# VinAIResearch/COMBAT

Hardware: AMD Instinct MI355X
Metric: images/sec per alternated generator+surrogate step, CIFAR-10 bs=128, 1/2/4/8 GPU (higher is better)
Workload: dtype bf16; 1 GPU; train_generator.py --dataset cifar10 --pc 0.5 --noise_rate 0.08: alternated PreActResNet18 surrogate + UNet generator step (Phase C + Phase G, both Nesterov-SGD updates), bs=128 per GPU, on-device augmentation on; per_gpu_batch=128, global_batch=128, parallelism=dp1 (RCCL all-reduce of netC grads in Phase C, netG grads in Phase G), losses_finite=True, deterministic=True

## Files before the change

### combat_amd/csrc/common.hpp

```cpp
#pragma once
#include <hip/hip_runtime.h>
#include <hip/hip_ext.h>
#include <stdint.h>

#include "combat_hip.h"

typedef __attribute__((ext_vector_type(8))) __bf16 bf16x8_t;
typedef __attribute__((ext_vector_type(4))) float f32x4_t;
typedef __attribute__((ext_vector_type(4))) short s16x4_t;
typedef __attribute__((ext_vector_type(4))) unsigned int u32x4_t;

namespace combat_launch {
extern thread_local hipEvent_t t_stop;
extern thread_local bool t_stop_used;
}
#define COMBAT_LAUNCH(kernel, grid, block, smem, stream, ...)                                             \
    do {                                                                                                  \
        if (hipEvent_t stop_ = combat_launch::t_stop) {                                                   \
            hipExtLaunchKernelGGL(kernel, grid, block, smem, stream, nullptr, stop_, 0, __VA_ARGS__);     \
            combat_launch::t_stop_used = true;                                                            \
        } else {                                                                                          \
            hipLaunchKernelGGL(kernel, grid, block, smem, stream, __VA_ARGS__);                           \
        }                                                                                                 \
    } while (0)
// ... 33 lines not shown
    v[4] = bf16_bits_to_f32(u[2] & 0xffffu);
    v[5] = bf16_bits_to_f32(u[2] >> 16);
    v[6] = bf16_bits_to_f32(u[3] & 0xffffu);
    v[7] = bf16_bits_to_f32(u[3] >> 16);
}

__device__ __forceinline__ u32x4_t pack8v(const float (&v)[8]) {
    u32x4_t u;
    u[0] = pack_bf16x2(v[0], v[1]);
    u[1] = pack_bf16x2(v[2], v[3]);
    u[2] = pack_bf16x2(v[4], v[5]);
    u[3] = pack_bf16x2(v[6], v[7]);
    return u;
}

__device__ __forceinline__ uint4 pack8(const float (&v)[8]) {
    uint4 u;
    u.x = pack_bf16x2(v[0], v[1]);
    u.y = pack_bf16x2(v[2], v[3]);
    u.z = pack_bf16x2(v[4], v[5]);
    u.w = pack_bf16x2(v[6], v[7]);
    return u;
}

__device__ __forceinline__ void load8f(const float *p, float (&v)[8]) {
    const float4 a = *reinterpret_cast<const float4 *>(p);
    const float4 b = *reinterpret_cast<const float4 *>(p + 4);
    v[0] = a.x; v[1] = a.y; v[2] = a.z; v[3] = a.w;
    v[4] = b.x; v[5] = b.y; v[6] = b.z; v[7] = b.w;
}

__device__ __forceinline__ float round_bf16(float f) { return bf16_bits_to_f32(f32_to_bf16_bits(f)); }

__device__ __forceinline__ uint4 hilo_pixel(float r, float g, float b) {
    const float hr = round_bf16(r), hg = round_bf16(g), hb = round_bf16(b);
    uint4 u;
    u.x = pack_bf16x2(hr, hg);
    u.y = pack_bf16x2(hb, r - hr);
    u.z = pack_bf16x2(g - hg, b - hb);
    u.w = 0;
    return u;
}

static inline hipStream_t as_stream(void *s) { return reinterpret_cast<hipStream_t>(s); }

bool combat_deterministic();
float *combat_stream_scratch(void *stream, size_t bytes);

static inline int ilog2_exact(int v) {
    if (v <= 0 || (v & (v - 1))) return -1;
    int s = 0;
    while ((1 << s) < v) ++s;
    return s;
}
```

### combat_amd/csrc/conv_wgrad.hip

```cpp
#include "conv_common.hpp"
#include "plan.hpp"

namespace {

struct WgradParams {
    combat_wgrad_args a;
    int M, PQ, ntaps, tiles_k, tiles_c, split, pix_per_split;
    float *ws;
};

template <int BMC, int BNC>
struct WCfg {
    static constexpr int WGK = (BNC == 16) ? 4 : (BMC == 16 ? 1 : 2);
    static constexpr int WGC = 4 / WGK;
    static constexpr int WK = BMC / WGK;
    static constexpr int WC = BNC / WGC;
    static constexpr int FK = WK / 16;
    static constexpr int FC = WC / 16;
    static constexpr int SK = (BMC + 16) * 2;
    static constexpr int SC = (BNC + 16) * 2;
    static constexpr int CHK = BMC / 8;
    static constexpr int CHC = BNC / 8;
    static constexpr int ITK = (64 * CHK + 255) / 256;
    static constexpr int ITC = (64 * CHC + 255) / 256;
// ... 168 lines not shown
#pragma unroll
        for (int i = 0; i < T::FK; ++i)
#pragma unroll
            for (int j = 0; j < T::FC; ++j) {
                const int col = wave_c * T::WC + j * 16 + fr;
                const int row = wave_k * T::WK + i * 16 + fq * 4;
#pragma unroll
                for (int e = 0; e < 4; ++e) ep[(row + e) * T::EPS + col] = acc[i][j][e];
            }
    }
    __syncthreads();
    if (p.ws) {
        float *slab = p.ws + ((((size_t)sp * p.ntaps + tap) * p.tiles_k + tile_k) * p.tiles_c + tile_c) * (size_t)(BMC * BNC);
        for (int idx = tid; idx < BMC * BNC; idx += 256) {
            const int row = idx / BNC, col = idx - row * BNC;
            slab[idx] = ep[row * T::EPS + col];
        }
        return;
    }
    const int creal = a.c_real;
    for (int idx = tid; idx < BMC * BNC; idx += 256) {
        const int row = idx / BNC, col = idx - row * BNC;
        const int n = k0 + row;
        int c = c0 + col;
        if (n >= a.k_real || c >= C) continue;
        if (creal < C) {
            if (c >= 2 * creal) continue;
            if (c >= creal) c -= creal;
        }
        atomicAdd(a.dw + ((size_t)n * p.ntaps + tap) * creal + c, ep[row * T::EPS + col]);
    }
}

__global__ __launch_bounds__(256) void conv_wgrad_c8_kernel(const WgradParams p) {
    constexpr int BMC = 64, NCOL = 80, SK = (BMC + 16) * 2, SC = (NCOL + 16) * 2, BUF = 64 * (SK + SC);
    constexpr int CHK = BMC / 8, CHC = NCOL / 8, ITK = (64 * CHK + 255) / 256, ITC = (64 * CHC + 255) / 256;
    constexpr int FC = NCOL / 16, EPS = NCOL + 4;
    extern __shared__ __attribute__((aligned(16))) unsigned char smem[];
    const combat_wgrad_args &a = p.a;
    const int tid = threadIdx.x, lane = tid & 63, wid = tid >> 6;
    int bid = blockIdx.x;
    const int tile_k = bid % p.tiles_k;
    const int sp = bid / p.tiles_k;
    const int k0 = tile_k * BMC;
    const int m_begin = sp * p.pix_per_split;
    int m_end = m_begin + p.pix_per_split;
    if (m_end > p.M) m_end = p.M;
    const int nkt = (m_end - m_begin + 63) / 64;
    if (nkt <= 0) return;
    const __bf16 *__restrict__ src = reinterpret_cast<const __bf16 *>(a.src);
    const __bf16 *__restrict__ dy = reinterpret_cast<const __bf16 *>(a.dy);
    const int K = a.K, H = a.H, W = a.W;
    u32x4_t rk[ITK];
    uint4 rc[ITC];
    auto load_tile = [&](int kt) {
        const int mt = m_begin + kt * 64;
#pragma unroll
        for (int i = 0; i < ITK; ++i) {
            const int idx = tid + 256 * i;
            const int row = idx / CHK, ch = idx % CHK;
            const int m = mt + row;
            u32x4_t v = {0u, 0u, 0u, 0u};
            if (idx < 64 * CHK && m < m_end) v = *reinterpret_cast<const u32x4_t *>(dy + (size_t)m * K + k0 + ch * 8);
            rk[i] = v;
        }
#pragma unroll
        for (int i = 0; i < ITC; ++i) {
            const int idx = tid + 256 * i;
            const int row = idx / CHC, tap = idx % CHC;
            const int m = mt + row;
            uint4 v = make_uint4(0, 0, 0, 0);
            if (idx < 64 * CHC && m < m_end && tap < 9) {
                const int img = m / p.PQ, rem = m - img * p.PQ;
                const int oy = rem / a.Q, ox = rem - oy * a.Q;
                const int r = (tap * 11) >> 5, s = tap - r * 3;
                const int iy = oy * a.stride - a.pad + r, ix = ox * a.stride - a.pad + s;
                if ((unsigned)iy < (unsigned)H && (unsigned)ix < (unsigned)W)
                    v = *reinterpret_cast<const uint4 *>(src + ((size_t)(img * H + iy) * W + ix) * 8);
            }
            rc[i] = v;
        }
    };
    auto store_tile = [&](int buf) {
        unsigned char *kl = smem + buf * BUF;
        unsigned char *cl = kl + 64 * SK;
#pragma unroll
        for (int i = 0; i < ITK; ++i) {
            const int idx = tid + 256 * i;
            if (idx < 64 * CHK) *reinterpret_cast<u32x4_t *>(kl + (idx / CHK) * SK + (idx % CHK) * 16) = rk[i];
        }
#pragma unroll
        for (int i = 0; i < ITC; ++i) {
            const int idx = tid + 256 * i;
            if (idx < 64 * CHC) *reinterpret_cast<uint4 *>(cl + (idx / CHC) * SC + (idx % CHC) * 16) = rc[i];
        }
    };
    f32x4_t acc[FC];
#pragma unroll
    for (int j = 0; j < FC; ++j) acc[j] = f32x4_t{0.f, 0.f, 0.f, 0.f};
    auto compute = [&](int buf) {
        const unsigned char *kl = smem + buf * BUF;
        const unsigned char *cl = kl + 64 * SK;
        const int q = (lane & 15) >> 2, pp = lane & 3, fq = lane >> 4;
        typedef __attribute__((ext_vector_type(8))) short s16x8_t;
        bf16x8_t fk[2], fc[2][FC];
#pragma unroll
        for (int ks = 0; ks < 2; ++ks) {
            const int prow = ks * 32 + fq * 8 + q;
            {
                const unsigned char *b = kl + prow * SK + (wid * 16 + pp * 4) * 2;
                const s16x4_t lo = lds_tr16(b), hi = lds_tr16(b + 4 * SK);
                const s16x8_t v = {lo[0], lo[1], lo[2], lo[3], hi[0], hi[1], hi[2], hi[3]};
                fk[ks] = __builtin_bit_cast(bf16x8_t, v);
            }
#pragma unroll
            for (int j = 0; j < FC; ++j) {
                const unsigned char *b = cl + prow * SC + (j * 16 + pp * 4) * 2;
                const s16x4_t lo = lds_tr16(b), hi = lds_tr16(b + 4 * SC);
                const s16x8_t v = {lo[0], lo[1], lo[2], lo[3], hi[0], hi[1], hi[2], hi[3]};
                fc[ks][j] = __builtin_bit_cast(bf16x8_t, v);
            }
        }
        __builtin_amdgcn_sched_barrier(0);
#pragma unroll
        for (int ks = 0; ks < 2; ++ks)
#pragma unroll
            for (int j = 0; j < FC; ++j) acc[j] = __builtin_amdgcn_mfma_f32_16x16x32_bf16(fk[ks], fc[ks][j], acc[j], 0, 0, 0);
        __builtin_amdgcn_sched_barrier(0);
    };
    load_tile(0);
    store_tile(0);
    __syncthreads();
    for (int kt = 0; kt < nkt; ++kt) {
        const bool more = kt + 1 < nkt;
        if (more) load_tile(kt + 1);
        compute(kt & 1);
        if (more) store_tile((kt + 1) & 1);
        __syncthreads();
    }
    float *ep = reinterpret_cast<float *>(smem);
    {
        const int fr = lane & 15, fq = lane >> 4;
#pragma unroll
        for (int j = 0; j < FC; ++j) {
            const int col = j * 16 + fr, row = wid * 16 + fq * 4;
#pragma unroll
            for (int e = 0; e < 4; ++e) ep[(row + e) * EPS + col] = acc[j][e];
        }
    }
    __syncthreads();
    const int creal = a.c_real;
    if (p.ws) {
        float *slab = p.ws + (size_t)blockIdx.x * (BMC * 9 * creal);
        for (int idx = tid; idx < BMC * 9 * creal; idx += 256) {
            const int row = idx / (9 * creal), rem = idx - row * 9 * creal;
            const int tap = rem / creal, c = rem - tap * creal;
            float v = ep[row * EPS + tap * 8 + c];
            if (creal < 8 && c + creal < 8) v += ep[row * EPS + tap * 8 + c + creal];
            slab[idx] = v;
        }
        return;
    }
    for (int idx = tid; idx < BMC * 72; idx += 256) {
        const int row = idx / 72, col = idx - row * 72;
        const int n = k0 + row, tap = col >> 3;
        int c = col & 7;
        if (n >= a.k_real) continue;
        if (creal < 8) {
            if (c >= 2 * creal) continue;
            if (c >= creal) c -= creal;
        }
        atomicAdd(a.dw + ((size_t)n * 9 + tap) * creal + c, ep[row * EPS + col]);
    }
}

__global__ __launch_bounds__(256) void conv_wgrad_c8_reduce_kernel(const float *__restrict__ ws, float *__restrict__ dw,
                                                                   int tiles_k, int split, int per_tile, int k_real,
                                                                   int row_elems, float *__restrict__ part) {
    const int e = blockIdx.x * 256 + threadIdx.x, tile_k = blockIdx.y;
    if (e >= per_tile) return;
    const int n = tile_k * 64 + e / row_elems;
    if (n >= k_real) return;
    float s0 = 0.f, s1 = 0.f, s2 = 0.f, s3 = 0.f;
    const int G = gridDim.z;
    int sp = blockIdx.z;
    for (; sp + 3 * G < split; sp += 4 * G) {
        s0 += ws[((size_t)sp * tiles_k + tile_k) * per_tile + e];
        s1 += ws[((size_t)(sp + G) * tiles_k + tile_k) * per_tile + e];
        s2 += ws[((size_t)(sp + 2 * G) * tiles_k + tile_k) * per_tile + e];
        s3 += ws[((size_t)(sp + 3 * G) * tiles_k + tile_k) * per_tile + e];
    }
    for (; sp < split; sp += G) s0 += ws[((size_t)sp * tiles_k + tile_k) * per_tile + e];
    const float s = (s0 + s1) + (s2 + s3);
    if (part) part[((size_t)blockIdx.z * tiles_k + tile_k) * per_tile + e] = s;
    else atomicAdd(dw + (size_t)tile_k * per_tile + e, s);
}

int launch_c8(WgradParams p, hipStream_t st) {
    constexpr int SMEM = 2 * 64 * ((64 + 16) * 2 + (80 + 16) * 2);
    static_assert(SMEM >= 64 * 84 * 4, "epilogue image");
    static bool attr_set = false;
    if (!attr_set) {
        if (hipFuncSetAttribute(reinterpret_cast<const void *>(conv_wgrad_c8_kernel), hipFuncAttributeMaxDynamicSharedMemorySize, SMEM) != hipSuccess)
            return COMBAT_ELAUNCH;
        attr_set = true;
    }
    p.tiles_k = p.a.K / 64;
    p.tiles_c = 1;
    int split = p.a.split;
    const int ktiles = (p.M + 63) / 64;
    if (split <= 0) {
        split = (256 + p.tiles_k - 1) / p.tiles_k;
        const int max_split = (ktiles + 3) / 4;
        if (split > max_split) split = max_split;
        if (split < 1) split = 1;
    }
    if (split > ktiles) split = ktiles;
    p.pix_per_split = ((ktiles + split - 1) / split) * 64;
    p.split = (p.M + p.pix_per_split - 1) / p.pix_per_split;
    const int per_tile = 64 * 9 * p.a.c_real;
    const long need = (long)p.tiles_k * p.split * per_tile * 4;
    p.ws = (p.split > 1 && p.a.workspace && p.a.workspace_bytes >= need) ? reinterpret_cast<float *>(p.a.workspace) : nullptr;
    if (combat_deterministic() && p.split > 1 && !p.ws) return COMBAT_EINVAL;
    COMBAT_LAUNCH(conv_wgrad_c8_kernel, dim3((unsigned)(p.tiles_k * p.split)), dim3(256), SMEM, st, p);
    CB_LAUNCH_CHECK();
    if (p.ws) {
        const int groups = p.split >= 32 ? 16 : 1;
        float *part = nullptr;
        if (combat_deterministic() && groups > 1) {
            const long extra = (long)groups * p.tiles_k * per_tile * 4;
            if (p.a.workspace_bytes >= need + extra) part = p.ws + need / 4;
        }
        const int g1 = combat_deterministic() && !part ? 1 : groups;
        COMBAT_LAUNCH(conv_wgrad_c8_reduce_kernel, dim3((per_tile + 255) / 256, p.tiles_k, g1), dim3(256), 0, st, (const float *)p.ws,
                           p.a.dw, p.tiles_k, p.split, per_tile, p.a.k_real, 9 * p.a.c_real, part);
        CB_LAUNCH_CHECK();
        if (part) {
            COMBAT_LAUNCH(conv_wgrad_c8_reduce_kernel, dim3((per_tile + 255) / 256, p.tiles_k, 1), dim3(256), 0, st, (const float *)part,
                               p.a.dw, p.tiles_k, groups, per_tile, p.a.k_real, 9 * p.a.c_real, (float *)nullptr);
            CB_LAUNCH_CHECK();
        }
    }
    return COMBAT_OK;
}

__global__ __launch_bounds__(256) void wgrad_slab_reduce_kernel(const float *__restrict__ ws, float *__restrict__ dw, int split,
                                                                int ntaps, int tiles_k, int tiles_c, int bmc, int bnc, int k_real,
                                                                int c_real, int C) {
    const long e = (long)blockIdx.x * 256 + threadIdx.x;
    if (e >= (long)k_real * ntaps * c_real) return;
    const int c = (int)(e % c_real), tap = (int)((e / c_real) % ntaps), n = (int)(e / ((long)c_real * ntaps));
    const int tile_k = n / bmc, row = n - tile_k * bmc;
    const size_t tile_elems = (size_t)bmc * bnc, sstride = (size_t)ntaps * tiles_k * tiles_c * tile_elems;
    float total = 0.f;
    for (int half = 0; half < 2; ++half) {
        const int cs = c + half * c_real;
        if (half && (c_real >= C || cs >= C || cs >= 2 * c_real)) break;
        const int tile_c = cs / bnc, col = cs - tile_c * bnc;
        const float *src = ws + (((size_t)tap * tiles_k + tile_k) * tiles_c + tile_c) * tile_elems + (size_t)row * bnc + col;
        float s0 = 0.f, s1 = 0.f, s2 = 0.f, s3 = 0.f;
        int sp = 0;
        for (; sp + 4 <= split; sp += 4) {
            s0 += src[(size_t)sp * sstride];
            s1 += src[(size_t)(sp + 1) * sstride];
            s2 += src[(size_t)(sp + 2) * sstride];
            s3 += src[(size_t)(sp + 3) * sstride];
        }
        for (; sp < split; ++sp) s0 += src[(size_t)sp * sstride];
        total += (s0 + s1) + (s2 + s3);
    }
    dw[e] += total;
}
// ... 39 lines not shown
    COMBAT_LAUNCH(kern, dim3((unsigned)blocks), dim3(256), T::SMEM, st, p);
    CB_LAUNCH_CHECK();
    if (p.ws) {
        const long elems = (long)p.a.k_real * p.ntaps * p.a.c_real;
        COMBAT_LAUNCH(wgrad_slab_reduce_kernel, dim3((unsigned)((elems + 255) / 256)), dim3(256), 0, st, (const float *)p.ws, p.a.dw,
                      p.split, p.ntaps, p.tiles_k, p.tiles_c, BMC, BNC, p.a.k_real, p.a.c_real, p.a.C);
        CB_LAUNCH_CHECK();
    }
    return COMBAT_OK;
}

template <int BMC, int BNC>
int generic_split(const combat_wgrad_args &a) {
    const long M = (long)a.N * a.P * a.Q;
    const int ktiles = (int)((M + 63) / 64), ntaps = a.R * a.S;
    const int tiles_k = (a.K + BMC - 1) / BMC, tiles_c = (a.C + BNC - 1) / BNC;
    int split = a.split > 0 ? a.split : 0;
    if (split <= 0) {
        const int base = tiles_k * tiles_c * ntaps;
        split = ((BMC == 16 ? 2304 : 256) + base - 1) / base;
        const int max_split = (ktiles + 3) / 4;
        if (split > max_split) split = max_split;
        if (split < 1) split = 1;
    }
    if (split > ktiles) split = ktiles;
    const int pix_per_split = ((ktiles + split - 1) / split) * 64;
    return (int)((M + pix_per_split - 1) / pix_per_split);
}

bool c8_applies(const combat_wgrad_args *a) {
    return a->split >= 0 && a->C == 8 && a->R == 3 && (a->K & 63) == 0 && !a->pro_scale && !a->pro_act;
}

int64_t c8_workspace(const combat_wgrad_args &a) {
    const long M = (long)a.N * a.P * a.Q;
    const int ktiles = (int)((M + 63) / 64), tiles_k = a.K / 64;
    int split = a.split;
    if (split <= 0) {
        split = (256 + tiles_k - 1) / tiles_k;
        const int max_split = (ktiles + 3) / 4;
        if (split > max_split) split = max_split;
        if (split < 1) split = 1;
    }
    if (split > ktiles) split = ktiles;
    const int pix_per_split = ((ktiles + split - 1) / split) * 64;
    const long nsplit = (M + pix_per_split - 1) / pix_per_split;
    if (nsplit <= 1) return 0;
    const int64_t per_tile = 64 * 9 * a.c_real * 4;
    return tiles_k * nsplit * per_tile + (nsplit >= 32 ? 16 * tiles_k * per_tile : 0);
}

int64_t generic_workspace(const combat_wgrad_args &a) {
    if (a.C <= 16) return generic_slab_bytes<64, 16>(a, generic_split<64, 16>(a));
    if (a.K <= 16) return generic_slab_bytes<16, 64>(a, generic_split<16, 64>(a));
    if (a.C % 128 == 0 && a.K % 128 == 0) return generic_slab_bytes<128, 128>(a, generic_split<128, 128>(a));
    return generic_slab_bytes<64, 64>(a, generic_split<64, 64>(a));
}

}

extern "C" int64_t combat_conv_wgrad_workspace_bytes(const combat_wgrad_args *a) {
    if (!a) return 0;
    const int64_t dma = a->split >= 0 ? (int64_t)conv_wgrad3x3_dma_workspace(a) : 0;
    if (dma > 0 || !combat_deterministic()) return dma;
    return c8_applies(a) ? c8_workspace(*a) : generic_workspace(*a);
}
// ... 27 lines not shown

extern "C" int combat_conv_wgrad_group(const combat_wgrad_args *const *members, int32_t n, void *workspace, int64_t workspace_bytes,
                                       void *stream) {
    COMBAT_PLAN_HOOK(combat_conv_wgrad_group, members, n, workspace, workspace_bytes);
    if (!members || n < 1) return COMBAT_EINVAL;
    for (int i = 0; i < n; ++i)
        if (validate_wgrad_args(members[i]) != COMBAT_OK) return COMBAT_EINVAL;
    return conv_wgrad3x3_dma_group(members, n, workspace, (long)workspace_bytes, as_stream(stream));
}

extern "C" int combat_conv_wgrad(const combat_wgrad_args *a, void *stream) {
    COMBAT_PLAN_HOOK(combat_conv_wgrad, a);
    if (validate_wgrad_args(a) != COMBAT_OK) return COMBAT_EINVAL;
    WgradParams p;
    p.a = *a;
    p.ws = nullptr;
    p.PQ = a->P * a->Q;
    p.M = (int)((long)a->N * p.PQ);
    p.ntaps = a->R * a->S;
    hipStream_t st = as_stream(stream);
    if (a->split >= 0) {
        int rc = conv_wgrad3x3_dma_try(a, st);
        if (rc <= 0) return rc;
    }
    if (a->reduce_first) {
        const int rc = combat_conv_wgrad_reduce(a->reduce_first, stream);
        if (rc != COMBAT_OK) return rc;
    }
    if (a->split >= 0 && !combat_deterministic()) {
        const int rc = conv_wgrad3x3_try(a, st);
        if (rc <= 0) return rc;
    }
    if (a->split < 0) p.a.split = 0;
    if (c8_applies(a)) return launch_c8(p, st);
    if (a->C <= 16) return launch<64, 16>(p, st);
    if (a->K <= 16) return launch<16, 64>(p, st);
    if (a->C % 128 == 0 && a->K % 128 == 0) return launch<128, 128>(p, st);
    return launch<64, 64>(p, st);
}
```

### combat_amd/csrc/elementwise.hip

```cpp
#include "common.hpp"
#include "plan.hpp"

namespace {

__global__ __launch_bounds__(256) void pack_weights_kernel(const float *__restrict__ w, int K, int taps, int creal,
                                                           int C, int dup, __bf16 *__restrict__ wf, int rows_f,
                                                           int kpad_f, __bf16 *__restrict__ wd, int rows_d,
                                                           int kpad_d, int Kc) {
    const long nf = (long)rows_f * kpad_f;
    const long nd = wd ? (long)rows_d * kpad_d : 0;
    for (long t = (long)blockIdx.x * blockDim.x + threadIdx.x; t < nf + nd; t += (long)gridDim.x * blockDim.x) {
        if (t < nf) {
            const int n = (int)(t / kpad_f), k = (int)(t - (long)n * kpad_f);
            const int tap = k / C, c = k - tap * C;
            float v = 0.f;
            if (n < K && tap < taps) {
                int cm = -1;
                if (c < creal) cm = c;
                else if (dup && c < 2 * creal) cm = c - creal;
                if (cm >= 0) v = w[((long)n * taps + tap) * creal + cm];
            }
            wf[t] = (__bf16)v;
        } else {
            const long u = t - nf;
// ... 259 lines not shown
    const int nch = a.C >> 3, Ho = 2 * a.H, Wo = 2 * a.W;
    const long total = (long)a.N * Ho * Wo * nch;
    for (long t = (long)blockIdx.x * blockDim.x + threadIdx.x; t < total; t += (long)gridDim.x * blockDim.x) {
        const int c = (int)(t % nch) * 8;
        long p = t / nch;
        const int ox = (int)(p % Wo);
        p /= Wo;
        const int oy = (int)(p % Ho);
        const long img = p / Ho;
        int y0, y1, x0, x1;
        float wy0, wy1, wx0, wx1;
        up_taps(oy, a.H, y0, y1, wy0, wy1);
        up_taps(ox, a.W, x0, x1, wx0, wx1);
        float u00[8], u01[8], u10[8], u11[8], o[8];
        u_value(a, img, y0, x0, c, u00);
        u_value(a, img, y0, x1, c, u01);
        u_value(a, img, y1, x0, c, u10);
        u_value(a, img, y1, x1, c, u11);
#pragma unroll
        for (int e = 0; e < 8; ++e) {
            const float v = wy0 * (wx0 * u00[e] + wx1 * u01[e]) + wy1 * (wx0 * u10[e] + wx1 * u11[e]);
            o[e] = v > 0.f ? v : 0.2f * v;
        }
        *reinterpret_cast<uint4 *>(a.out + ((img * Ho + oy) * Wo + ox) * a.C + c) = pack8(o);
    }
}

__global__ __launch_bounds__(256) void unet_up_bwd_kernel(const __bf16 *__restrict__ d_out,
                                                          const __bf16 *__restrict__ out, int N, int H, int W, int C,
                                                          __bf16 *__restrict__ du) {
    const int nch = C >> 3, Ho = 2 * H, Wo = 2 * W;
    const long total = (long)N * H * W * nch;
    for (long t = (long)blockIdx.x * blockDim.x + threadIdx.x; t < total; t += (long)gridDim.x * blockDim.x) {
        const int c = (int)(t % nch) * 8;
        long p = t / nch;
        const int ix = (int)(p % W);
        p /= W;
        const int iy = (int)(p % H);
        const long img = p / H;
        float acc[8];
#pragma unroll
        for (int e = 0; e < 8; ++e) acc[e] = 0.f;
        for (int oy = 2 * iy - 1; oy <= 2 * iy + 2; ++oy) {
            if (oy < 0 || oy >= Ho) continue;
            int y0, y1;
            float wy0, wy1;
            up_taps(oy, H, y0, y1, wy0, wy1);
            const float wy = (y0 == iy ? wy0 : 0.f) + (y1 == iy ? wy1 : 0.f);
            if (wy == 0.f) continue;
            for (int ox = 2 * ix - 1; ox <= 2 * ix + 2; ++ox) {
                if (ox < 0 || ox >= Wo) continue;
                int x0, x1;
                float wx0, wx1;
                up_taps(ox, W, x0, x1, wx0, wx1);
                const float wx = (x0 == ix ? wx0 : 0.f) + (x1 == ix ? wx1 : 0.f);
                if (wx == 0.f) continue;
                const long off = ((img * Ho + oy) * Wo + ox) * C + c;
                float g[8], o[8];
                unpack8(*reinterpret_cast<const uint4 *>(d_out + off), g);
                unpack8(*reinterpret_cast<const uint4 *>(out + off), o);
                const float wgt = wy * wx;
#pragma unroll
                for (int e = 0; e < 8; ++e) acc[e] = fmaf(wgt * (o[e] > 0.f ? 1.f : 0.2f), g[e], acc[e]);
            }
        }
        *reinterpret_cast<uint4 *>(du + ((img * H + iy) * W + ix) * C + c) = pack8(acc);
    }
}

__global__ __launch_bounds__(256) void sgd_kernel(void *const *__restrict__ ptrs, const int64_t *__restrict__ sizes,
                                                  float lr, float mu, float wd, float gscale, int first) {
    const int t = blockIdx.y;
    float *__restrict__ p = reinterpret_cast<float *>(ptrs[3 * t]);
    const float *__restrict__ g = reinterpret_cast<const float *>(ptrs[3 * t + 1]);
    float *__restrict__ b = reinterpret_cast<float *>(ptrs[3 * t + 2]);
    const long n = sizes[t];
    for (long i = (long)blockIdx.x * blockDim.x + threadIdx.x; i < n; i += (long)gridDim.x * blockDim.x) {
        const float pv = p[i];
        const float gv = fmaf(wd, pv, g[i] * gscale);
        const float bv = first ? gv : fmaf(mu, b[i], gv);
        b[i] = bv;
        p[i] = pv - lr * fmaf(mu, bv, gv);
    }
}

__global__ __launch_bounds__(256) void linear_nhwc_kernel(const __bf16 *__restrict__ x, int h, int w, int C,
                                                          const float *__restrict__ Wt, const float *__restrict__ b,
                                                          int classes, float *__restrict__ logits) {
    __shared__ float red[256];
    const int img = blockIdx.x;
    const int in = C * h * w;
    for (int j = 0; j < classes; ++j) {
        float s = 0.f;
        for (int i = threadIdx.x; i < in; i += 256) {
            const int c = i / (h * w), r = i - c * h * w;
            s = fmaf((float)x[((long)img * h * w + r) * C + c], Wt[(long)j * in + i], s);
        }
        red[threadIdx.x] = s;
// ... 404 lines not shown
```

### combat_amd/csrc/norm.hip

```cpp
#include "common.hpp"
#include "plan.hpp"

namespace {

constexpr int kStageRows = 64;

__device__ __forceinline__ void reduce_rows(const float *__restrict__ part, int C, int c, long row0, int nrows,
                                            int ry, double &s1, double &s2) {
    s1 = 0.0;
    s2 = 0.0;
    if (c >= C) return;
    for (int r = ry; r < nrows; r += 32) {
        float u[8], v[8];
#pragma unroll
        for (int q = 0; q < 8; ++q) {
            const int rr = r + 4 * q < nrows ? r + 4 * q : r;
            const float *p = part + ((row0 + rr) * 2) * (long)C + c;
            u[q] = p[0];
            v[q] = p[C];
        }
#pragma unroll
        for (int q = 0; q < 8; ++q) {
            if (r + 4 * q < nrows) {
                s1 += (double)u[q];
// ... 471 lines not shown
    for (long ib = i0 + pl; ib < i1; ib += 32 * NB) {
        if (ib != i0 + pl) load_pass(ib);
#pragma unroll
        for (int q = 0; q < NB; ++q) {
            const long i = ib + 32 * q;
            if (i >= i1) break;
            const long off = ((long)g * a.pxg + i) * a.C + c;
            float dv[8], xv[8], o[8];
            unpack8v(ld[q], dv);
            unpack8v(lx[q], xv);
#pragma unroll
            for (int e = 0; e < 8; ++e) o[e] = fmaf(ka[e], dv[e], fmaf(kb[e], xv[e], kc[e]));
            if (a.add) {
                float ad[8];
                unpack8v(la[q], ad);
#pragma unroll
                for (int e = 0; e < 8; ++e) o[e] += ad[e];
            }
            *reinterpret_cast<u32x4_t *>(a.dx + off) = pack8v(o);
        }
    }
}

struct UpFusedArgs {
    const __bf16 *y, *s;
    __bf16 *out;
    const float *part;
    int rpg, C, H, W, band;
    float eps;
    const float *ss, *ts;
    float *mean, *rstd, *scale, *shift;
};

__device__ __forceinline__ void up_taps2(int o, int n, int &i0, int &i1, float &w0, float &w1) {
    const int i = o >> 1;
    if (o & 1) {
        i0 = i;
        i1 = i + 1 < n ? i + 1 : n - 1;
        w0 = 0.75f;
        w1 = 0.25f;
    } else {
        i0 = i > 0 ? i - 1 : 0;
        i1 = i;
        w0 = 0.25f;
        w1 = 0.75f;
    }
}

__global__ __launch_bounds__(256) void unet_up_fused_kernel(const UpFusedArgs a) {
    const int tid = threadIdx.x, co = tid & 7, pl = tid >> 3;
    const int c = blockIdx.x * 64 + co * 8, band = blockIdx.y, g = blockIdx.z;
    const bool live = c < a.C;
    const long pxg = (long)a.H * a.W;
    double s1[8], s2[8];
#pragma unroll
    for (int e = 0; e < 8; ++e) s1[e] = s2[e] = 0.0;
    if (live) {
        if (a.part) {
            for (int r = pl; r < a.rpg; r += 32) {
                const float *p = a.part + (((long)g * a.rpg + r) * 2) * a.C + c;
                float u[8], v[8];
                load8f(p, u);
                load8f(p + a.C, v);
#pragma unroll
                for (int e = 0; e < 8; ++e) {
                    s1[e] += (double)u[e];
                    s2[e] += (double)v[e];
                }
            }
        } else {
            float f1[8], f2[8];
#pragma unroll
            for (int e = 0; e < 8; ++e) f1[e] = f2[e] = 0.f;
            for (long i = pl; i < pxg; i += 32) {
                float v[8];
                unpack8(*reinterpret_cast<const uint4 *>(a.y + ((long)g * pxg + i) * a.C + c), v);
#pragma unroll
                for (int e = 0; e < 8; ++e) {
                    f1[e] += v[e];
// ... 12 lines not shown
    fused_combine(s1, s2, tid, sums);
    if (tid < 64) {
        const int cc = blockIdx.x * 64 + tid;
        double t1, t2;
        fused_channel_sums(sums, tid, t1, t2);
        const double cnt = (double)pxg, mean = t1 / cnt;
        double var = t2 / cnt - mean * mean;
        if (var < 0.0) var = 0.0;
        const double rstd = 1.0 / sqrt(var + (double)a.eps);
        const float fsc = (float)rstd, fsh = (float)(-mean * rstd);
        coef[0][tid] = fsc;
        coef[1][tid] = fsh;
        if (cc < a.C && band == 0) {
            const long o = (long)g * a.C + cc;
            if (a.mean) a.mean[o] = (float)mean;
            if (a.rstd) a.rstd[o] = (float)rstd;
            if (a.scale) a.scale[o] = fsc;
            if (a.shift) a.shift[o] = fsh;
        }
    }
    __syncthreads();
    if (!live) return;
    float sy[8], ty[8], ss[8], ts[8];
#pragma unroll
    for (int e = 0; e < 8; ++e) {
        sy[e] = coef[0][co * 8 + e];
        ty[e] = coef[1][co * 8 + e];
        ss[e] = ts[e] = 0.f;
    }
    if (a.s) {
        load8f(a.ss + (long)g * a.C + c, ss);
        load8f(a.ts + (long)g * a.C + c, ts);
    }
    const int Ho = 2 * a.H, Wo = 2 * a.W;
    const int oy0 = band * a.band, oy1 = oy0 + a.band < Ho ? oy0 + a.band : Ho;
    auto u_at = [&](int iy, int ix, float (&u)[8]) {
        const long off = (((long)g * a.H + iy) * a.W + ix) * a.C + c;
        float v[8];
        unpack8(*reinterpret_cast<const uint4 *>(a.y + off), v);
#pragma unroll
        for (int e = 0; e < 8; ++e) u[e] = fmaf(v[e], sy[e], ty[e]);
        if (a.s) {
            unpack8(*reinterpret_cast<const uint4 *>(a.s + off), v);
#pragma unroll
            for (int e = 0; e < 8; ++e) {
                const float q = fmaf(v[e], ss[e], ts[e]);
                u[e] += q > 0.f ? q : 0.2f * q;
            }
        }
    };
    for (int p = oy0 * Wo + pl; p < oy1 * Wo; p += 32) {
        const int oy = p / Wo, ox = p - oy * Wo;
        int y0, y1, x0, x1;
        float wy0, wy1, wx0, wx1;
        up_taps2(oy, a.H, y0, y1, wy0, wy1);
        up_taps2(ox, a.W, x0, x1, wx0, wx1);
        float u00[8], u01[8], u10[8], u11[8], o[8];
        u_at(y0, x0, u00);
        u_at(y0, x1, u01);
        u_at(y1, x0, u10);
        u_at(y1, x1, u11);
#pragma unroll
        for (int e = 0; e < 8; ++e) {
            const float v = wy0 * (wx0 * u00[e] + wx1 * u01[e]) + wy1 * (wx0 * u10[e] + wx1 * u11[e]);
            o[e] = v > 0.f ? v : 0.2f * v;
        }
        *reinterpret_cast<uint4 *>(a.out + (((long)g * Ho + oy) * Wo + ox) * a.C + c) = pack8(o);
    }
}

__device__ __forceinline__ float up_adjoint_weight(int i, int n, int k) {
    if (k == 0) return i >= 1 ? 0.25f : 0.f;
    if (k == 1) return i == 0 ? 1.f : 0.75f;
    if (k == 2) return i == n - 1 ? 1.f : 0.75f;
    return i + 1 < n ? 0.25f : 0.f;
}

struct UpBwdFusedArgs {
    const __bf16 *d_out, *out, *y;
    __bf16 *du, *dx;
    int C, H, W;
    const float *mean, *rstd;
};

__global__ __launch_bounds__(256) void unet_up_bwd_fused_kernel(const UpBwdFusedArgs a) {
    const int tid = threadIdx.x, co = tid & 7, pl = tid >> 3;
    const int c = blockIdx.x * 64 + co * 8, g = blockIdx.y;
    const bool live = c < a.C;
    const int H = a.H, W = a.W, Ho = 2 * H, Wo = 2 * W;
    const long pxg = (long)H * W;
    float mu[8], rs[8], f1[8], f2[8];
#pragma unroll
    for (int e = 0; e < 8; ++e) {
        mu[e] = f1[e] = f2[e] = 0.f;
        rs[e] = 1.f;
    }
    if (live) {
        load8f(a.mean + (long)g * a.C + c, mu);
        load8f(a.rstd + (long)g * a.C + c, rs);
        for (long i = pl; i < pxg; i += 32) {
            const int iy = (int)(i / W), ix = (int)(i - (long)iy * W);
            float acc[8], wx[4];
            int oxc[4];
#pragma unroll
            for (int e = 0; e < 8; ++e) acc[e] = 0.f;
#pragma unroll
            for (int k = 0; k < 4; ++k) {
                const int ox = 2 * ix - 1 + k;
                wx[k] = up_adjoint_weight(ix, W, k);
// ... 184 lines not shown
                                     int64_t px_per_group, int32_t C, float eps, float slope, const float *gamma,
                                     const float *beta, float *mean, float *rstd, float *scale, float *shift,
                                     float *running_mean, float *running_var, float momentum,
                                     int64_t *num_batches_tracked, float *scratch, int64_t scratch_bytes, void *act,
                                     void *stream) {
    COMBAT_PLAN_HOOK(combat_norm_act_fused, x, partials, groups, rows_per_group, px_per_group, C, eps, slope, gamma, beta, mean, rstd, scale, shift, running_mean, running_var, momentum, num_batches_tracked, scratch, scratch_bytes, act);
    return norm_act_fused_launch(x, partials, groups, rows_per_group, px_per_group, C, eps, slope, gamma, beta, mean, rstd,
                                 scale, shift, running_mean, running_var, momentum, num_batches_tracked, scratch,
                                 scratch_bytes, nullptr, nullptr, nullptr, act, stream);
}

extern "C" int combat_norm_add_act_fused(const void *x, const float *partials, int32_t groups, int32_t rows_per_group,
                                         int64_t px_per_group, int32_t C, float eps, float slope, const float *gamma,
                                         const float *beta, float *mean, float *rstd, float *scale, float *shift,
                                         float *running_mean, float *running_var, float momentum,
                                         int64_t *num_batches_tracked, float *scratch, int64_t scratch_bytes,
                                         const void *add, const float *add_scale, const float *add_shift, void *act,
                                         void *stream) {
    COMBAT_PLAN_HOOK(combat_norm_add_act_fused, x, partials, groups, rows_per_group, px_per_group, C, eps, slope, gamma, beta, mean, rstd, scale, shift, running_mean, running_var, momentum, num_batches_tracked, scratch, scratch_bytes, add, add_scale, add_shift, act);
    if (!add) return COMBAT_EINVAL;
    return norm_act_fused_launch(x, partials, groups, rows_per_group, px_per_group, C, eps, slope, gamma, beta, mean, rstd,
                                 scale, shift, running_mean, running_var, momentum, num_batches_tracked, scratch,
                                 scratch_bytes, add, add_scale, add_shift, act, stream);
}

extern "C" int combat_unet_up_fused(const void *y, const float *partials, int32_t rows_per_group, const void *s,
                                    const float *ss, const float *ts, int32_t N, int32_t H, int32_t W, int32_t C,
                                    float eps, float *mean, float *rstd, float *scale, float *shift, void *out,
                                    void *stream) {
    COMBAT_PLAN_HOOK(combat_unet_up_fused, y, partials, rows_per_group, s, ss, ts, N, H, W, C, eps, mean, rstd, scale, shift, out);
    if (!y || !out || N <= 0 || H <= 0 || W <= 0 || C <= 0 || (C & 7)) return COMBAT_EINVAL;
    if (s && (!ss || !ts)) return COMBAT_EINVAL;
    if (partials ? (rows_per_group <= 0 || rows_per_group > kFusedMaxRows) : (long)H * W > kFusedMaxDirect) return COMBAT_EINVAL;
    const int wg_c = (C + 63) / 64, Ho = 2 * H, Wo = 2 * W;
    int bands = 1;
    while ((long)N * wg_c * bands < 512 && bands * 2 <= Ho && (Ho / (bands * 2)) * Wo >= 32) bands *= 2;
    const int band = (Ho + bands - 1) / bands;
    UpFusedArgs a{reinterpret_cast<const __bf16 *>(y), reinterpret_cast<const __bf16 *>(s), reinterpret_cast<__bf16 *>(out),
                  partials, partials ? rows_per_group : 0, C, H, W, band, eps, ss, ts, mean, rstd, scale, shift};
    COMBAT_LAUNCH(unet_up_fused_kernel, dim3(wg_c, (Ho + band - 1) / band, N), dim3(256), 0, as_stream(stream), a);
    CB_LAUNCH_CHECK();
    return COMBAT_OK;
}

extern "C" int combat_unet_up_bwd_fused(const void *d_out, const void *out, const void *y, const float *mean,
                                        const float *rstd, int32_t N, int32_t H, int32_t W, int32_t C, void *du,
                                        void *dx, void *stream) {
    COMBAT_PLAN_HOOK(combat_unet_up_bwd_fused, d_out, out, y, mean, rstd, N, H, W, C, du, dx);
    if (!d_out || !out || !y || !mean || !rstd || !du || !dx || N <= 0 || H <= 0 || W <= 0 || C <= 0 || (C & 7))
        return COMBAT_EINVAL;
    if ((long)H * W > kFusedMaxDirect) return COMBAT_EINVAL;
    UpBwdFusedArgs a{reinterpret_cast<const __bf16 *>(d_out), reinterpret_cast<const __bf16 *>(out),
                     reinterpret_cast<const __bf16 *>(y), reinterpret_cast<__bf16 *>(du), reinterpret_cast<__bf16 *>(dx),
                     C, H, W, mean, rstd};
    COMBAT_LAUNCH(unet_up_bwd_fused_kernel, dim3((C + 63) / 64, N), dim3(256), 0, as_stream(stream), a);
    CB_LAUNCH_CHECK();
    return COMBAT_OK;
}

extern "C" int combat_norm_bwd_fused(const void *dz, const void *x, const void *add, const float *partials,
                                     int32_t groups, int32_t rows_per_group, int64_t px_per_group, int32_t C,
                                     const float *gamma, const float *mean, const float *rstd, float *dgamma,
                                     float *dbeta, float *scratch, int64_t scratch_bytes, void *dx, void *stream) {
    COMBAT_PLAN_HOOK(combat_norm_bwd_fused, dz, x, add, partials, groups, rows_per_group, px_per_group, C, gamma, mean, rstd, dgamma, dbeta, scratch, scratch_bytes, dx);
    if (!dz || !x || !dx || !mean || !rstd || groups <= 0 || px_per_group <= 0 || C <= 0 || (C & 7))
        return COMBAT_EINVAL;
    if (partials ? rows_per_group <= 0 : px_per_group > kFusedMaxDirect) return COMBAT_EINVAL;
    if ((dgamma || dbeta) && groups != 1) return COMBAT_EINVAL;
    hipStream_t st = as_stream(stream);
    int rpg = partials ? rows_per_group : 0;
    const float *src = partials;
    if (partials && rpg > kFusedMaxRows) {
        int err;
// ... 76 lines not shown
```

Measured before the change: 33900 images/sec.

## Add K8 wgrad path and restructure bilinear upsample forward/adjoint kernels

Adds a wgrad variant for 8-output-channel 3x3 convs that tiles over input channels, fusing the prologue affine and activation. It is disabled in deterministic mode. Rewrites the fused upsample kernel to process one input pixel per thread, reusing a 3x3 neighbourhood to emit four output pixels instead of reloading four neighbours per output. Rewrites the upsample adjoint kernel with branch-free unrolled 4x4 gathers and 32-bit index math. This trades extra register pressure for fewer redundant loads and divisions.

Result: no change. 33930 images/sec, median of 5 (+0.1%).

```diff
diff --git a/combat_amd/csrc/common.hpp b/combat_amd/csrc/common.hpp
--- a/combat_amd/csrc/common.hpp
+++ b/combat_amd/csrc/common.hpp
@@ -89,6 +89,13 @@
 
 __device__ __forceinline__ float round_bf16(float f) { return bf16_bits_to_f32(f32_to_bf16_bits(f)); }
 
+__device__ __forceinline__ float up_adjoint_weight(int i, int n, int k) {
+    if (k == 0) return i >= 1 ? 0.25f : 0.f;
+    if (k == 1) return i == 0 ? 1.f : 0.75f;
+    if (k == 2) return i == n - 1 ? 1.f : 0.75f;
+    return i + 1 < n ? 0.25f : 0.f;
+}
+
 __device__ __forceinline__ uint4 hilo_pixel(float r, float g, float b) {
     const float hr = round_bf16(r), hg = round_bf16(g), hb = round_bf16(b);
     uint4 u;
diff --git a/combat_amd/csrc/conv_wgrad.hip b/combat_amd/csrc/conv_wgrad.hip
--- a/combat_amd/csrc/conv_wgrad.hip
+++ b/combat_amd/csrc/conv_wgrad.hip
@@ -224,6 +224,7 @@
     }
 }
 
+template <bool K8>
 __global__ __launch_bounds__(256) void conv_wgrad_c8_kernel(const WgradParams p) {
     constexpr int BMC = 64, NCOL = 80, SK = (BMC + 16) * 2, SC = (NCOL + 16) * 2, BUF = 64 * (SK + SC);
     constexpr int CHK = BMC / 8, CHC = NCOL / 8, ITK = (64 * CHK + 255) / 256, ITC = (64 * CHC + 255) / 256;
@@ -232,8 +233,9 @@
     const combat_wgrad_args &a = p.a;
     const int tid = threadIdx.x, lane = tid & 63, wid = tid >> 6;
     int bid = blockIdx.x;
-    const int tile_k = bid % p.tiles_k;
-    const int sp = bid / p.tiles_k;
+    const int tiles = K8 ? p.tiles_c : p.tiles_k;
+    const int tile_k = bid % tiles;
+    const int sp = bid / tiles;
     const int k0 = tile_k * BMC;
     const int m_begin = sp * p.pix_per_split;
     int m_end = m_begin + p.pix_per_split;
@@ -243,17 +245,31 @@
     const __bf16 *__restrict__ src = reinterpret_cast<const __bf16 *>(a.src);
     const __bf16 *__restrict__ dy = reinterpret_cast<const __bf16 *>(a.dy);
     const int K = a.K, H = a.H, W = a.W;
+    const __bf16 *__restrict__ rows = K8 ? src : dy;
+    const int row_stride = K8 ? a.C : K;
+    const bool pro_affine = K8 && a.pro_scale != nullptr, pro_act = K8 && a.pro_act;
     u32x4_t rk[ITK];
     uint4 rc[ITC];
+    unsigned vk = 0;
+    int gk[ITK], gcur = -1;
+    float psc[8], psh[8];
     auto load_tile = [&](int kt) {
         const int mt = m_begin + kt * 64;
+        vk = 0;
 #pragma unroll
         for (int i = 0; i < ITK; ++i) {
             const int idx = tid + 256 * i;
             const int row = idx / CHK, ch = idx % CHK;
             const int m = mt + row;
             u32x4_t v = {0u, 0u, 0u, 0u};
-            if (idx < 64 * CHK && m < m_end) v = *reinterpret_cast<const u32x4_t *>(dy + (size_t)m * K + k0 + ch * 8);
+            gk[i] = 0;
+            if (idx < 64 * CHK && m < m_end) {
+                v = *reinterpret_cast<const u32x4_t *>(rows + (size_t)m * row_stride + k0 + ch * 8);
+                if (K8) {
+                    vk |= 1u << i;
+                    if (a.pro_group_stride) gk[i] = (m / p.PQ) * a.pro_group_stride;
+                }
+            }
             rk[i] = v;
         }
 #pragma unroll
@@ -266,9 +282,9 @@
                 const int img = m / p.PQ, rem = m - img * p.PQ;
                 const int oy = rem / a.Q, ox = rem - oy * a.Q;
                 const int r = (tap * 11) >> 5, s = tap - r * 3;
-                const int iy = oy * a.stride - a.pad + r, ix = ox * a.stride - a.pad + s;
+                const int iy = K8 ? oy + 1 - r : oy * a.stride - a.pad + r, ix = K8 ? ox + 1 - s : ox * a.stride - a.pad + s;
                 if ((unsigned)iy < (unsigned)H && (unsigned)ix < (unsigned)W)
-                    v = *reinterpret_cast<const uint4 *>(src + ((size_t)(img * H + iy) * W + ix) * 8);
+                    v = *reinterpret_cast<const uint4 *>((K8 ? dy : src) + ((size_t)(img * H + iy) * W + ix) * 8);
             }
             rc[i] = v;
         }
@@ -279,7 +295,28 @@
 #pragma unroll
         for (int i = 0; i < ITK; ++i) {
             const int idx = tid + 256 * i;
-            if (idx < 64 * CHK) *reinterpret_cast<u32x4_t *>(kl + (idx / CHK) * SK + (idx % CHK) * 16) = rk[i];
+            if (idx < 64 * CHK) {
+                u32x4_t val = rk[i];
+                if (K8 && (pro_affine || pro_act) && ((vk >> i) & 1u)) {
+                    float v[8];
+                    unpack8(__builtin_bit_cast(uint4, val), v);
+                    if (pro_affine) {
+                        if (gk[i] != gcur) {
+                            gcur = gk[i];
+                            load8f(a.pro_scale + gcur + k0 + (idx % CHK) * 8, psc);
+                            load8f(a.pro_shift + gcur + k0 + (idx % CHK) * 8, psh);
+                        }
+#pragma unroll
+                        for (int e = 0; e < 8; ++e) v[e] = fmaf(v[e], psc[e], psh[e]);
+                    }
+                    if (pro_act) {
+#pragma unroll
+                        for (int e = 0; e < 8; ++e) v[e] = v[e] > 0.f ? v[e] : v[e] * a.pro_slope;
+                    }
+                    val = __builtin_bit_cast(u32x4_t, pack8(v));
+                }
+                *reinterpret_cast<u32x4_t *>(kl + (idx / CHK) * SK + (idx % CHK) * 16) = val;
+            }
         }
 #pragma unroll
         for (int i = 0; i < ITC; ++i) {
@@ -342,6 +379,17 @@
     }
     __syncthreads();
     const int creal = a.c_real;
+    if (K8) {
+        float *slab = p.ws ? p.ws + (size_t)blockIdx.x * (8 * 9 * BMC) : nullptr;
+        for (int idx = tid; idx < 8 * 9 * BMC; idx += 256) {
+            const int k = idx / (9 * BMC), rem = idx - k * 9 * BMC;
+            const int tap = rem / BMC, c = rem - tap * BMC;
+            const float v = ep[c * EPS + tap * 8 + k];
+            if (slab) slab[idx] = v;
+            else if (k < a.k_real && k0 + c < creal) atomicAdd(a.dw + ((size_t)k * 9 + tap) * creal + k0 + c, v);
+        }
+        return;
+    }
     if (p.ws) {
         float *slab = p.ws + (size_t)blockIdx.x * (BMC * 9 * creal);
         for (int idx = tid; idx < BMC * 9 * creal; idx += 256) {
@@ -366,13 +414,20 @@
     }
 }
 
+template <bool K8>
 __global__ __launch_bounds__(256) void conv_wgrad_c8_reduce_kernel(const float *__restrict__ ws, float *__restrict__ dw,
                                                                    int tiles_k, int split, int per_tile, int k_real,
-                                                                   int row_elems, float *__restrict__ part) {
+                                                                   int row_elems, int creal, float *__restrict__ part) {
     const int e = blockIdx.x * 256 + threadIdx.x, tile_k = blockIdx.y;
     if (e >= per_tile) return;
-    const int n = tile_k * 64 + e / row_elems;
+    const int n = K8 ? e / row_elems : tile_k * 64 + e / row_elems;
     if (n >= k_real) return;
+    size_t out = (size_t)tile_k * per_tile + e;
+    if (K8) {
+        const int c = tile_k * 64 + (e & 63);
+        if (c >= creal) return;
+        out = (size_t)(e >> 6) * creal + c;
+    }
     float s0 = 0.f, s1 = 0.f, s2 = 0.f, s3 = 0.f;
     const int G = gridDim.z;
     int sp = blockIdx.z;
@@ -385,24 +440,26 @@
     for (; sp < split; sp += G) s0 += ws[((size_t)sp * tiles_k + tile_k) * per_tile + e];
     const float s = (s0 + s1) + (s2 + s3);
     if (part) part[((size_t)blockIdx.z * tiles_k + tile_k) * per_tile + e] = s;
-    else atomicAdd(dw + (size_t)tile_k * per_tile + e, s);
-}
-
+    else atomicAdd(dw + out, s);
+}
+
+template <bool K8>
 int launch_c8(WgradParams p, hipStream_t st) {
     constexpr int SMEM = 2 * 64 * ((64 + 16) * 2 + (80 + 16) * 2);
     static_assert(SMEM >= 64 * 84 * 4, "epilogue image");
     static bool attr_set = false;
     if (!attr_set) {
-        if (hipFuncSetAttribute(reinterpret_cast<const void *>(conv_wgrad_c8_kernel), hipFuncAttributeMaxDynamicSharedMemorySize, SMEM) != hipSuccess)
+        if (hipFuncSetAttribute(reinterpret_cast<const void *>(conv_wgrad_c8_kernel<K8>), hipFuncAttributeMaxDynamicSharedMemorySize, SMEM) != hipSuccess)
             return COMBAT_ELAUNCH;
         attr_set = true;
     }
-    p.tiles_k = p.a.K / 64;
-    p.tiles_c = 1;
+    const int tiles = K8 ? p.a.C / 64 : p.a.K / 64;
+    p.tiles_k = K8 ? 1 : tiles;
+    p.tiles_c = K8 ? tiles : 1;
     int split = p.a.split;
     const int ktiles = (p.M + 63) / 64;
     if (split <= 0) {
-        split = (256 + p.tiles_k - 1) / p.tiles_k;
+        split = (256 + tiles - 1) / tiles;
         const int max_split = (ktiles + 3) / 4;
         if (split > max_split) split = max_split;
         if (split < 1) split = 1;
@@ -410,26 +467,27 @@
     if (split > ktiles) split = ktiles;
     p.pix_per_split = ((ktiles + split - 1) / split) * 64;
     p.split = (p.M + p.pix_per_split - 1) / p.pix_per_split;
-    const int per_tile = 64 * 9 * p.a.c_real;
-    const long need = (long)p.tiles_k * p.split * per_tile * 4;
+    const int per_tile = K8 ? 8 * 9 * 64 : 64 * 9 * p.a.c_real;
+    const int row_elems = K8 ? 9 * 64 : 9 * p.a.c_real;
+    const long need = (long)tiles * p.split * per_tile * 4;
     p.ws = (p.split > 1 && p.a.workspace && p.a.workspace_bytes >= need) ? reinterpret_cast<float *>(p.a.workspace) : nullptr;
     if (combat_deterministic() && p.split > 1 && !p.ws) return COMBAT_EINVAL;
-    COMBAT_LAUNCH(conv_wgrad_c8_kernel, dim3((unsigned)(p.tiles_k * p.split)), dim3(256), SMEM, st, p);
+    COMBAT_LAUNCH(conv_wgrad_c8_kernel<K8>, dim3((unsigned)(tiles * p.split)), dim3(256), SMEM, st, p);
     CB_LAUNCH_CHECK();
     if (p.ws) {
         const int groups = p.split >= 32 ? 16 : 1;
         float *part = nullptr;
         if (combat_deterministic() && groups > 1) {
-            const long extra = (long)groups * p.tiles_k * per_tile * 4;
+            const long extra = (long)groups * tiles * per_tile * 4;
             if (p.a.workspace_bytes >= need + extra) part = p.ws + need / 4;
         }
         const int g1 = combat_deterministic() && !part ? 1 : groups;
-        COMBAT_LAUNCH(conv_wgrad_c8_reduce_kernel, dim3((per_tile + 255) / 256, p.tiles_k, g1), dim3(256), 0, st, (const float *)p.ws,
-                           p.a.dw, p.tiles_k, p.split, per_tile, p.a.k_real, 9 * p.a.c_real, part);
+        COMBAT_LAUNCH(conv_wgrad_c8_reduce_kernel<K8>, dim3((per_tile + 255) / 256, tiles, g1), dim3(256), 0, st, (const float *)p.ws,
+                           p.a.dw, tiles, p.split, per_tile, p.a.k_real, row_elems, p.a.c_real, part);
         CB_LAUNCH_CHECK();
         if (part) {
-            COMBAT_LAUNCH(conv_wgrad_c8_reduce_kernel, dim3((per_tile + 255) / 256, p.tiles_k, 1), dim3(256), 0, st, (const float *)part,
-                               p.a.dw, p.tiles_k, groups, per_tile, p.a.k_real, 9 * p.a.c_real, (float *)nullptr);
+            COMBAT_LAUNCH(conv_wgrad_c8_reduce_kernel<K8>, dim3((per_tile + 255) / 256, tiles, 1), dim3(256), 0, st, (const float *)part,
+                               p.a.dw, tiles, groups, per_tile, p.a.k_real, row_elems, p.a.c_real, (float *)nullptr);
             CB_LAUNCH_CHECK();
         }
     }
@@ -535,6 +593,10 @@
     return a->split >= 0 && a->C == 8 && a->R == 3 && (a->K & 63) == 0 && !a->pro_scale && !a->pro_act;
 }
 
+bool k8_applies(const combat_wgrad_args *a) {
+    return !combat_deterministic() && a->split >= 0 && a->K == 8 && a->R == 3 && a->stride == 1 && a->pad == 1 && a->P == a->H && a->Q == a->W && (a->C & 63) == 0;
+}
+
 int64_t c8_workspace(const combat_wgrad_args &a) {
     const long M = (long)a.N * a.P * a.Q;
     const int ktiles = (int)((M + 63) / 64), tiles_k = a.K / 64;
@@ -628,8 +690,9 @@
         if (rc <= 0) return rc;
     }
     if (a->split < 0) p.a.split = 0;
-    if (c8_applies(a)) return launch_c8(p, st);
+    if (c8_applies(a)) return launch_c8<false>(p, st);
     if (a->C <= 16) return launch<64, 16>(p, st);
+    if (k8_applies(a)) return launch_c8<true>(p, st);
     if (a->K <= 16) return launch<16, 64>(p, st);
     if (a->C % 128 == 0 && a->K % 128 == 0) return launch<128, 128>(p, st);
     return launch<64, 64>(p, st);
diff --git a/combat_amd/csrc/elementwise.hip b/combat_amd/csrc/elementwise.hip
--- a/combat_amd/csrc/elementwise.hip
+++ b/combat_amd/csrc/elementwise.hip
@@ -315,38 +315,60 @@
     const int nch = C >> 3, Ho = 2 * H, Wo = 2 * W;
     const long total = (long)N * H * W * nch;
     for (long t = (long)blockIdx.x * blockDim.x + threadIdx.x; t < total; t += (long)gridDim.x * blockDim.x) {
-        const int c = (int)(t % nch) * 8;
-        long p = t / nch;
-        const int ix = (int)(p % W);
-        p /= W;
-        const int iy = (int)(p % H);
-        const long img = p / H;
+        int c, ix, iy;
+        long img;
+        if (total <= 0x7fffffffL) {
+            const unsigned tt = (unsigned)t, p = tt / (unsigned)nch, q = p / (unsigned)W;
+            c = (int)(tt - p * nch) * 8;
+            ix = (int)(p - q * W);
+            img = q / (unsigned)H;
+            iy = (int)(q - (unsigned)img * H);
+        } else {
+            c = (int)(t % nch) * 8;
+            long p = t / nch;
+            ix = (int)(p % W);
+            p /= W;
+            iy = (int)(p % H);
+            img = p / H;
+        }
+        float wy[4], wx[4];
+        long row[4];
+        int col[4];
+#pragma unroll
+        for (int k = 0; k < 4; ++k) {
+            const int oy = 2 * iy - 1 + k, ox = 2 * ix - 1 + k;
+            wy[k] = up_adjoint_weight(iy, H, k);
+            wx[k] = up_adjoint_weight(ix, W, k);
+            row[k] = (img * Ho + (oy < 0 ? 0 : (oy >= Ho ? Ho - 1 : oy))) * Wo;
+            col[k] = ox < 0 ? 0 : (ox >= Wo ? Wo - 1 : ox);
+        }
+        uint4 gq[4][4], oq[4][4];
+#pragma unroll
+        for (int ky = 0; ky < 4; ++ky)
+#pragma unroll
+            for (int kx = 0; kx < 4; ++kx) {
+                const long off = (row[ky] + col[kx]) * C + c;
+                gq[ky][kx] = *reinterpret_cast<const uint4 *>(d_out + off);
+                oq[ky][kx] = *reinterpret_cast<const uint4 *>(out + off);
+            }
         float acc[8];
 #pragma unroll
         for (int e = 0; e < 8; ++e) acc[e] = 0.f;
-        for (int oy = 2 * iy - 1; oy <= 2 * iy + 2; ++oy) {
-            if (oy < 0 || oy >= Ho) continue;
-            int y0, y1;
-            float wy0, wy1;
-            up_taps(oy, H, y0, y1, wy0, wy1);
-            const float wy = (y0 == iy ? wy0 : 0.f) + (y1 == iy ? wy1 : 0.f);
-            if (wy == 0.f) continue;
-            for (int ox = 2 * ix - 1; ox <= 2 * ix + 2; ++ox) {
-                if (ox < 0 || ox >= Wo) continue;
-                int x0, x1;
-                float wx0, wx1;
-                up_taps(ox, W, x0, x1, wx0, wx1);
-                const float wx = (x0 == ix ? wx0 : 0.f) + (x1 == ix ? wx1 : 0.f);
-                if (wx == 0.f) continue;
-                const long off = ((img * Ho + oy) * Wo + ox) * C + c;
+#pragma unroll
+        for (int ky = 0; ky < 4; ++ky)
+#pragma unroll
+            for (int kx = 0; kx < 4; ++kx) {
+                const float wgt = wy[ky] * wx[kx];
+                const bool on = wgt != 0.f;
                 float g[8], o[8];
-                unpack8(*reinterpret_cast<const uint4 *>(d_out + off), g);
-                unpack8(*reinterpret_cast<const uint4 *>(out + off), o);
-                const float wgt = wy * wx;
-#pragma unroll
-                for (int e = 0; e < 8; ++e) acc[e] = fmaf(wgt * (o[e] > 0.f ? 1.f : 0.2f), g[e], acc[e]);
+                unpack8(gq[ky][kx], g);
+                unpack8(oq[ky][kx], o);
+#pragma unroll
+                for (int e = 0; e < 8; ++e) {
+                    const float v = fmaf(wgt * (o[e] > 0.f ? 1.f : 0.2f), g[e], acc[e]);
+                    acc[e] = on ? v : acc[e];
+                }
             }
-        }
         *reinterpret_cast<uint4 *>(du + ((img * H + iy) * W + ix) * C + c) = pack8(acc);
     }
 }
diff --git a/combat_amd/csrc/norm.hip b/combat_amd/csrc/norm.hip
--- a/combat_amd/csrc/norm.hip
+++ b/combat_amd/csrc/norm.hip
@@ -527,19 +527,15 @@
     float *mean, *rstd, *scale, *shift;
 };
 
-__device__ __forceinline__ void up_taps2(int o, int n, int &i0, int &i1, float &w0, float &w1) {
-    const int i = o >> 1;
-    if (o & 1) {
-        i0 = i;
-        i1 = i + 1 < n ? i + 1 : n - 1;
-        w0 = 0.75f;
-        w1 = 0.25f;
-    } else {
-        i0 = i > 0 ? i - 1 : 0;
-        i1 = i;
-        w0 = 0.25f;
-        w1 = 0.75f;
-    }
+__device__ __forceinline__ float up_bilerp(int e, float wy0, float wy1, float wx0, float wx1, float u00, float u01,
+                                           float u10, float u11) {
+#pragma clang fp contract(off)
+    if (e & 2) {
+        const float top = fmaf(wx0, u00, wx1 * u01), bot = fmaf(wx0, u10, wx1 * u11);
+        return fmaf(wy0, top, wy1 * bot);
+    }
+    const float bot = fmaf(wx1, u11, wx0 * u10), top = fmaf(wx1, u01, wx0 * u00);
+    return fmaf(wy1, bot, wy0 * top);
 }
 
 __global__ __launch_bounds__(256) void unet_up_fused_kernel(const UpFusedArgs a) {
@@ -618,49 +614,62 @@
         load8f(a.ss + (long)g * a.C + c, ss);
         load8f(a.ts + (long)g * a.C + c, ts);
     }
-    const int Ho = 2 * a.H, Wo = 2 * a.W;
-    const int oy0 = band * a.band, oy1 = oy0 + a.band < Ho ? oy0 + a.band : Ho;
-    auto u_at = [&](int iy, int ix, float (&u)[8]) {
-        const long off = (((long)g * a.H + iy) * a.W + ix) * a.C + c;
-        float v[8];
-        unpack8(*reinterpret_cast<const uint4 *>(a.y + off), v);
-#pragma unroll
-        for (int e = 0; e < 8; ++e) u[e] = fmaf(v[e], sy[e], ty[e]);
-        if (a.s) {
-            unpack8(*reinterpret_cast<const uint4 *>(a.s + off), v);
-#pragma unroll
-            for (int e = 0; e < 8; ++e) {
-                const float q = fmaf(v[e], ss[e], ts[e]);
-                u[e] += q > 0.f ? q : 0.2f * q;
-            }
-        }
-    };
-    for (int p = oy0 * Wo + pl; p < oy1 * Wo; p += 32) {
-        const int oy = p / Wo, ox = p - oy * Wo;
-        int y0, y1, x0, x1;
-        float wy0, wy1, wx0, wx1;
-        up_taps2(oy, a.H, y0, y1, wy0, wy1);
-        up_taps2(ox, a.W, x0, x1, wx0, wx1);
-        float u00[8], u01[8], u10[8], u11[8], o[8];
-        u_at(y0, x0, u00);
-        u_at(y0, x1, u01);
-        u_at(y1, x0, u10);
-        u_at(y1, x1, u11);
-#pragma unroll
-        for (int e = 0; e < 8; ++e) {
-            const float v = wy0 * (wx0 * u00[e] + wx1 * u01[e]) + wy1 * (wx0 * u10[e] + wx1 * u11[e]);
-            o[e] = v > 0.f ? v : 0.2f * v;
-        }
-        *reinterpret_cast<uint4 *>(a.out + (((long)g * Ho + oy) * Wo + ox) * a.C + c) = pack8(o);
-    }
-}
-
-__device__ __forceinline__ float up_adjoint_weight(int i, int n, int k) {
-    if (k == 0) return i >= 1 ? 0.25f : 0.f;
-    if (k == 1) return i == 0 ? 1.f : 0.75f;
-    if (k == 2) return i == n - 1 ? 1.f : 0.75f;
-    return i + 1 < n ? 0.25f : 0.f;
-}
+    const int H = a.H, W = a.W, Wo = 2 * W;
+    const int iy0 = band * a.band, rows = (iy0 + a.band < H ? iy0 + a.band : H) - iy0;
+    const int dq = 32 / W, dr = 32 - dq * W;
+    int r = pl / W, ix = pl - r * W;
+    for (; r < rows; r += dq, ix += dr) {
+        if (ix >= W) {
+            ix -= W;
+            if (++r >= rows) break;
+        }
+        const int iy = iy0 + r;
+        const int yy[3] = {iy > 0 ? iy - 1 : 0, iy, iy + 1 < H ? iy + 1 : H - 1};
+        const int xx[3] = {ix > 0 ? ix - 1 : 0, ix, ix + 1 < W ? ix + 1 : W - 1};
+        uint4 yq[3][3], sq[3][3];
+#pragma unroll
+        for (int j = 0; j < 3; ++j)
+#pragma unroll
+            for (int i = 0; i < 3; ++i) {
+                const long off = (((long)g * H + yy[j]) * W + xx[i]) * a.C + c;
+                yq[j][i] = *reinterpret_cast<const uint4 *>(a.y + off);
+                if (a.s) sq[j][i] = *reinterpret_cast<const uint4 *>(a.s + off);
+            }
+        float u[3][3][8];
+#pragma unroll
+        for (int j = 0; j < 3; ++j)
+#pragma unroll
+            for (int i = 0; i < 3; ++i) {
+                float v[8];
+                unpack8(yq[j][i], v);
+#pragma unroll
+                for (int e = 0; e < 8; ++e) u[j][i][e] = fmaf(v[e], sy[e], ty[e]);
+                if (a.s) {
+                    unpack8(sq[j][i], v);
+#pragma unroll
+                    for (int e = 0; e < 8; ++e) {
+                        const float q = fmaf(v[e], ss[e], ts[e]);
+                        u[j][i][e] += q > 0.f ? q : 0.2f * q;
+                    }
+                }
+            }
+#pragma unroll
+        for (int dy = 0; dy < 2; ++dy)
+#pragma unroll
+            for (int dx = 0; dx < 2; ++dx) {
+                const float wy0 = dy ? 0.75f : 0.25f, wy1 = dy ? 0.25f : 0.75f;
+                const float wx0 = dx ? 0.75f : 0.25f, wx1 = dx ? 0.25f : 0.75f;
+                float o[8];
+#pragma unroll
+                for (int e = 0; e < 8; ++e) {
+                    const float v = up_bilerp(e, wy0, wy1, wx0, wx1, u[dy][dx][e], u[dy][dx + 1][e], u[dy + 1][dx][e], u[dy + 1][dx + 1][e]);
+                    o[e] = v > 0.f ? v : 0.2f * v;
+                }
+                *reinterpret_cast<uint4 *>(a.out + (((long)g * 2 * H + 2 * iy + dy) * Wo + 2 * ix + dx) * a.C + c) = pack8(o);
+            }
+    }
+}
+
 
 struct UpBwdFusedArgs {
     const __bf16 *d_out, *out, *y;
@@ -911,13 +920,13 @@
     if (!y || !out || N <= 0 || H <= 0 || W <= 0 || C <= 0 || (C & 7)) return COMBAT_EINVAL;
     if (s && (!ss || !ts)) return COMBAT_EINVAL;
     if (partials ? (rows_per_group <= 0 || rows_per_group > kFusedMaxRows) : (long)H * W > kFusedMaxDirect) return COMBAT_EINVAL;
-    const int wg_c = (C + 63) / 64, Ho = 2 * H, Wo = 2 * W;
+    const int wg_c = (C + 63) / 64;
     int bands = 1;
-    while ((long)N * wg_c * bands < 512 && bands * 2 <= Ho && (Ho / (bands * 2)) * Wo >= 32) bands *= 2;
-    const int band = (Ho + bands - 1) / bands;
+    while ((long)N * wg_c * bands < 512 && bands * 2 <= H && (H / (bands * 2)) * W >= 16) bands *= 2;
+    const int band = (H + bands - 1) / bands;
     UpFusedArgs a{reinterpret_cast<const __bf16 *>(y), reinterpret_cast<const __bf16 *>(s), reinterpret_cast<__bf16 *>(out),
                   partials, partials ? rows_per_group : 0, C, H, W, band, eps, ss, ts, mean, rstd, scale, shift};
-    COMBAT_LAUNCH(unet_up_fused_kernel, dim3(wg_c, (Ho + band - 1) / band, N), dim3(256), 0, as_stream(stream), a);
+    COMBAT_LAUNCH(unet_up_fused_kernel, dim3(wg_c, (H + band - 1) / band, N), dim3(256), 0, as_stream(stream), a);
     CB_LAUNCH_CHECK();
     return COMBAT_OK;
 }
```
